# bmezaris/RetargetVid

Hardware: AMD Instinct MI355X
Metric: frames/sec end-to-end saliency+crop on 640x360 (higher is better)
Workload: dtype f32

## Files before the change

### retargetvid_amd/csrc/svc_net.hip

```cpp
#include <math.h>

#include <algorithm>

#include "svc_internal.h"
#include "svc_lanczos.h"
#include "svc_x3.h"

static inline int ceil_div(int a, int b) { return (a + b - 1) / b; }

__device__ __forceinline__ unsigned xcd_bx() {
    const unsigned b = blockIdx.x, n = gridDim.x;
    return (n & 7) ? b : (b & 7) * (n >> 3) + (b >> 3);
}

typedef float f32x2 __attribute__((ext_vector_type(2)));
__device__ __forceinline__ void fma4(float4 &a, const float4 x, const float4 w) {
    const f32x2 lo = __builtin_elementwise_fma((f32x2){x.x, x.y}, (f32x2){w.x, w.y}, (f32x2){a.x, a.y});
    const f32x2 hi = __builtin_elementwise_fma((f32x2){x.z, x.w}, (f32x2){w.z, w.w}, (f32x2){a.z, a.w});
    a = make_float4(lo.x, lo.y, hi.x, hi.y);
}


static thread_local char g_err[512] = "";
void svc_set_error(const char *fmt, ...) {
// ... 47 lines not shown
            const int ymin = vb[2 * y], cnt = vb[2 * y + 1];
            const int *k = vk + y * vks;
            const uint8_t *p = tile + (ymin - r_lo) * rowlen + i;
            int acc = 1 << (LZ_PREC - 1);
            for (int j = 0; j < cnt; ++j) acc += __mul24((int)p[j * rowlen], k[j]);
            dst[(size_t)(y - y0) * rowlen + i] = lc[min(max(acc >> LZ_PREC, 0), 255)];
        }
    }
}

#define STEM_TH 8
#define STEM_TW 16
#define STEM_PRS 100
__global__ __launch_bounds__(256) void k_stem_mfma(const float *__restrict__ X, const float *__restrict__ Wtr,
                                                   const float *__restrict__ bias, float *__restrict__ Y, int NH,
                                                   int NW, int OH, int OW, int tiles_x, int tiles_y) {
    constexpr int PR = 2 * STEM_TH + 1, PCW = 2 * STEM_TW + 1;
    __shared__ float Pin[PR * STEM_PRS];
    const int tid = threadIdx.x, lane = tid & 63, wave = tid >> 6, r = lane & 31, hh = lane >> 5;
    int bid = xcd_bx();
    const int tx = bid % tiles_x;
    bid /= tiles_x;
    const int ty = bid % tiles_y, f = bid / tiles_y;
    const int oy0 = ty * STEM_TH, ox0 = tx * STEM_TW, py0 = 2 * oy0 - 1, px0 = 2 * ox0 - 1;
    const float *xin = X + (size_t)f * NH * NW * 3;
    for (int idx = tid; idx < PR * PCW * 3; idx += 256) {
        const int pr = idx / (PCW * 3), rem = idx - pr * (PCW * 3), pc = rem / 3;
        const int y = py0 + pr, x = px0 + pc;
        float v = 0.f;
        if ((unsigned)y < (unsigned)NH && (unsigned)x < (unsigned)NW) v = xin[((long long)y * NW + px0) * 3 + rem];
        Pin[pr * STEM_PRS + rem] = v;
    }
    float4 wv[4];
#pragma unroll
    for (int q = 0; q < 4; ++q) wv[q] = *(const float4 *)(Wtr + r * 32 + 8 * q + 4 * hh);
    __syncthreads();
    const int p = 32 * wave + r, py = p / STEM_TW, px = p - py * STEM_TW;
    const float *src = Pin + (2 * py) * STEM_PRS + (2 * px) * 3;
    f32x16 acc;
#pragma unroll
    for (int i = 0; i < 16; ++i) acc[i] = 0.f;
#pragma unroll
    for (int q = 0; q < 4; ++q) {
        float t[4];
#pragma unroll
        for (int e = 0; e < 4; ++e) {
            const int k = 8 * q + 4 * hh + e;
            const int ky = (k * 57) >> 9;
            t[e] = k < 27 ? src[k + (STEM_PRS - 9) * ky] : 0.f;
        }
        acc = __builtin_amdgcn_mfma_f32_32x32x2f32(wv[q].x, t[0], acc, 0, 0, 0);
        acc = __builtin_amdgcn_mfma_f32_32x32x2f32(wv[q].y, t[1], acc, 0, 0, 0);
        acc = __builtin_amdgcn_mfma_f32_32x32x2f32(wv[q].z, t[2], acc, 0, 0, 0);
        acc = __builtin_amdgcn_mfma_f32_32x32x2f32(wv[q].w, t[3], acc, 0, 0, 0);
    }
    const int oy = oy0 + py, ox = ox0 + px;
    if (oy >= OH || ox >= OW) return;
    float *yp = Y + (((size_t)f * OH + oy) * OW + ox) * 32;
#pragma unroll
    for (int g = 0; g < 4; ++g) {
        const int c = 8 * g + 4 * hh;
        const float4 b = *(const float4 *)(bias + c);
        float4 v;
        v.x = fminf(fmaxf(acc[4 * g] + b.x, 0.f), 6.f);
        v.y = fminf(fmaxf(acc[4 * g + 1] + b.y, 0.f), 6.f);
        v.z = fminf(fmaxf(acc[4 * g + 2] + b.z, 0.f), 6.f);
        v.w = fminf(fmaxf(acc[4 * g + 3] + b.w, 0.f), 6.f);
        *(float4 *)(yp + c) = v;
    }
}

#define FR_TH 8
#define FR_TW 16
#define FR_HH (FR_TH + 2)
#define FR_HW (FR_TW + 2)
#define FR_NPX (FR_HH * FR_HW)
#define FR_PR (2 * FR_HH + 1)
#define FR_PC (2 * FR_HW + 1)
#define FR_PRS 112
#define FR_ES 36

#define FR_MAXT 32

struct FrontArgs {
    const uint8_t *frames;
    int h, w, NH, NW, OH, OW, tiles_x, tiles_y;
    const int *hb, *hk, *vb, *vk;
    int hks, vks;
    const float *lut;
    const float *Wstem, *bstem;
    const float *Wstem_l, *Wp_l;
    const float *Wd, *bd;
    const float *Wp, *bp;
    float *Y;
    float *in_dbg;
    int nr_cap, nc_cap;
    short row_lo[FR_MAXT], row_n[FR_MAXT], col_lo[FR_MAXT], col_n[FR_MAXT];
};

__host__ __device__ static inline int front_src_stride(int nc_cap) { return ((nc_cap * 3 + 6) >> 2) << 2; }
__host__ __device__ static inline int front_in_offset(int nr_cap, int nc_cap) {
    return (nr_cap * (front_src_stride(nc_cap) + FR_PRS) + 15) & ~15;
}
#define FR_IN_BYTES (FR_PR * FR_PRS * 4)
#define FR_SONLY_BYTES (FR_NPX * FR_ES * 4)
static inline int front_small_bytes(int nr_cap, int nc_cap) { return front_in_offset(nr_cap, nc_cap) + (FR_PR * 8 + 24 + 768) * 4; }
static inline int front_lds_bytes() { return FR_IN_BYTES + FR_SONLY_BYTES; }

__global__ __launch_bounds__(256) __attribute__((amdgpu_waves_per_eu(4, 8))) void k_front(const FrontArgs A) {
    extern __shared__ uint8_t sm_fr[];
    const int tid = threadIdx.x, lane = tid & 63, wave = tid >> 6, r = lane & 31, hh = lane >> 5;
    int bid = xcd_bx();
    const int tx = bid % A.tiles_x;
    bid /= A.tiles_x;
    const int ty = bid % A.tiles_y, f = bid / A.tiles_y;
    const int oy0 = ty * FR_TH, ox0 = tx * FR_TW, py0 = 2 * oy0 - 3, px0 = 2 * ox0 - 3;
    const int srs = front_src_stride(A.nc_cap);
    float *IN_s = (float *)sm_fr;
    float *S = (float *)(sm_fr + FR_IN_BYTES);
    uint8_t *src_s = (uint8_t *)S;
    uint8_t *tile_s = src_s + A.nr_cap * srs;
    int *vk_s = (int *)(src_s + front_in_offset(A.nr_cap, A.nc_cap));
    int *vb_s = vk_s + FR_PR * 8;
    float *lut_s = (float *)(vb_s + 24);
    float *D = S;
    const int c4 = tid & 7;
    const int ya = max(py0, 0), yb = min(py0 + FR_PR, A.NH), xa = max(px0, 0), xb = min(px0 + FR_PC, A.NW);
    const int r_lo = A.row_lo[ty], nr = A.row_n[ty], c_lo = A.col_lo[tx], nc3 = A.col_n[tx] * 3, ncol3 = (xb - xa) * 3;
    const uintptr_t g0 = (uintptr_t)A.frames + (((size_t)f * A.h + r_lo) * A.w + c_lo) * 3;
    const int rstep = A.w * 3, gm0 = (int)(g0 & 3), rs3 = rstep & 3;
    const int srow = tid >> 5, swi = tid & 31;
    uint32_t sv[4];
#pragma unroll
    for (int it = 0; it < 4; ++it) {
        const int row = srow + 8 * it;
        const uintptr_t ga = g0 + (size_t)row * rstep;
        const int nwords = ((int)(ga & 3) + nc3 + 3) >> 2;
        sv[it] = (row < nr && swi < nwords) ? *(const uint32_t *)((ga & ~(uintptr_t)3) + 4 * swi) : 0u;
    }
    const int ci = tid & 127, half = __builtin_amdgcn_readfirstlane(tid >> 7);
    const bool col_ok = ci < ncol3;
    const int xi = ci / 3, cc = ci - 3 * xi, x = min(xa + xi, A.NW - 1), pcol = (x - px0) * 3 + cc;
    const int xmin = A.hb[2 * x];
    int kh[8];
#pragma unroll
    for (int j = 0; j < 8; ++j) kh[j] = j < A.hks ? A.hk[x * A.hks + j] : 0;
    int vkv = 0, vbv = 0;
    if (tid < FR_PR * 8) {
        const int y = ya + (tid >> 3), j = tid & 7;
        if (y < yb && j < A.vks) vkv = A.vk[y * A.vks + j];
    } else if (tid < FR_PR * 8 + FR_PR) {
        const int y = ya + tid - FR_PR * 8;
        if (y < yb) vbv = A.vb[2 * y];
    }
    float lv[3];
#pragma unroll
    for (int i = 0; i < 3; ++i) lv[i] = A.lut[tid + 256 * i];
    for (int i = tid; i < FR_PR * FR_PRS / 4; i += 256) ((float4 *)IN_s)[i] = make_float4(0.f, 0.f, 0.f, 0.f);
#pragma unroll
    for (int it = 0; it < 4; ++it) {
        const int row = srow + 8 * it;
        if (row < nr && swi < (srs >> 2)) ((uint32_t *)src_s)[row * (srs >> 2) + swi] = sv[it];
    }
    if (tid < FR_PR * 8) vk_s[tid] = vkv;
    else if (tid < FR_PR * 8 + FR_PR) vb_s[tid - FR_PR * 8] = vbv;
#pragma unroll
    for (int i = 0; i < 3; ++i) lut_s[tid + 256 * i] = lv[i];
    __syncthreads();
    if (col_ok) {
        const uint8_t *p = src_s + (xmin - c_lo) * 3 + cc;
        for (int row = half; row < nr; row += 2) {
            const uint8_t *q = p + row * srs + ((gm0 + row * rs3) & 3);
            int acc = 1 << (LZ_PREC - 1);
#pragma unroll
            for (int j = 0; j < 8; ++j) acc += __mul24((int)q[3 * j], kh[j]);
            tile_s[row * FR_PRS + pcol] = (uint8_t)min(max(acc >> LZ_PREC, 0), 255);
        }
    }
    float4 wv[4];
#pragma unroll
    for (int q = 0; q < 4; ++q) wv[q] = *(const float4 *)(A.Wstem_l + (q * 64 + lane) * 4);
    __syncthreads();
    if (col_ok) {
        const float *lc = lut_s + cc * 256;
        const bool dbg_col = A.in_dbg && x >= 2 * ox0 && x < 2 * ox0 + 2 * FR_TW;
        for (int y = ya + half; y < yb; y += 2) {
            const int vrow = y - ya;
            const int4 k0 = *(const int4 *)(vk_s + vrow * 8), k1 = *(const int4 *)(vk_s + vrow * 8 + 4);
            const uint8_t *q = tile_s + (vb_s[vrow] - r_lo) * FR_PRS + pcol;
            int acc = 1 << (LZ_PREC - 1);
            acc += __mul24((int)q[0], k0.x) + __mul24((int)q[FR_PRS], k0.y) + __mul24((int)q[2 * FR_PRS], k0.z) + __mul24((int)q[3 * FR_PRS], k0.w);
            acc += __mul24((int)q[4 * FR_PRS], k1.x) + __mul24((int)q[5 * FR_PRS], k1.y) + __mul24((int)q[6 * FR_PRS], k1.z) + __mul24((int)q[7 * FR_PRS], k1.w);
            const float v = lc[min(max(acc >> LZ_PREC, 0), 255)];
            IN_s[(y - py0) * FR_PRS + pcol] = v;
            if (dbg_col && y >= 2 * oy0 && y < 2 * oy0 + 2 * FR_TH) A.in_dbg[(((size_t)f * A.NH + y) * A.NW + x) * 3 + cc] = v;
        }
    }
    __syncthreads();
    float4 wd[9];
#pragma unroll
    for (int t = 0; t < 9; ++t) wd[t] = *(const float4 *)(A.Wd + t * 32 + c4 * 4);
    for (int t = wave; t < (FR_NPX + 31) / 32; t += 4) {
        const int hp = t * 32 + r, hq = min(hp, FR_NPX - 1);
        const int hy = hq / FR_HW, hx = hq - hy * FR_HW;
        const float *src = IN_s + (2 * hy) * FR_PRS + (2 * hx) * 3;
        f32x16 acc;
#pragma unroll
        for (int i = 0; i < 16; ++i) acc[i] = 0.f;
#pragma unroll
        for (int q = 0; q < 4; ++q) {
            float tp[4];
#pragma unroll
            for (int e = 0; e < 4; ++e) {
                const int k = 8 * q + 4 * hh + e;
                const int ky = (k * 57) >> 9;
                tp[e] = k < 27 ? src[k + (FR_PRS - 9) * ky] : 0.f;
            }
            acc = __builtin_amdgcn_mfma_f32_32x32x2f32(wv[q].x, tp[0], acc, 0, 0, 0);
            acc = __builtin_amdgcn_mfma_f32_32x32x2f32(wv[q].y, tp[1], acc, 0, 0, 0);
            acc = __builtin_amdgcn_mfma_f32_32x32x2f32(wv[q].z, tp[2], acc, 0, 0, 0);
            acc = __builtin_amdgcn_mfma_f32_32x32x2f32(wv[q].w, tp[3], acc, 0, 0, 0);
        }
        if (hp < FR_NPX) {
            const bool in = (unsigned)(oy0 - 1 + hy) < (unsigned)A.OH && (unsigned)(ox0 - 1 + hx) < (unsigned)A.OW;
            float *sp = S + hp * FR_ES + 4 * hh;
#pragma unroll
            for (int g = 0; g < 4; ++g) {
                float4 v = make_float4(0.f, 0.f, 0.f, 0.f);
                if (in) {
                    const float4 b = *(const float4 *)(A.bstem + 8 * g + 4 * hh);
                    v.x = fminf(fmaxf(acc[4 * g] + b.x, 0.f), 6.f);
                    v.y = fminf(fmaxf(acc[4 * g + 1] + b.y, 0.f), 6.f);
                    v.z = fminf(fmaxf(acc[4 * g + 2] + b.z, 0.f), 6.f);
                    v.w = fminf(fmaxf(acc[4 * g + 3] + b.w, 0.f), 6.f);
                }
                *(float4 *)(sp + 8 * g) = v;
            }
        }
    }
    __syncthreads();
    float4 wq[4];
#pragma unroll
    for (int q = 0; q < 4; ++q) {
        wq[q] = *(const float4 *)(A.Wp_l + (q * 64 + lane) * 4);
        if (r >= 16) wq[q] = make_float4(0.f, 0.f, 0.f, 0.f);
    }
    {
        const float4 b = *(const float4 *)(A.bd + c4 * 4);
        const int oy = tid >> 5, ox = ((tid >> 3) & 3) * 4;
        float4 a4[4];
#pragma unroll
        for (int i = 0; i < 4; ++i) a4[i] = make_float4(0.f, 0.f, 0.f, 0.f);
#pragma unroll
        for (int ky = 0; ky < 3; ++ky) {
            const float *sp = S + ((oy + ky) * FR_HW + ox) * FR_ES + c4 * 4;
            float4 xv[6];
#pragma unroll
            for (int j = 0; j < 6; ++j) xv[j] = *(const float4 *)(sp + j * FR_ES);
#pragma unroll
            for (int kx = 0; kx < 3; ++kx) {
                const float4 w = wd[ky * 3 + kx];
#pragma unroll
                for (int i = 0; i < 4; ++i) fma4(a4[i], xv[i + kx], w);
            }
        }
        __syncthreads();
#pragma unroll
        for (int i = 0; i < 4; ++i) {
            float4 o;
            o.x = fminf(fmaxf(a4[i].x + b.x, 0.f), 6.f);
            o.y = fminf(fmaxf(a4[i].y + b.y, 0.f), 6.f);
            o.z = fminf(fmaxf(a4[i].z + b.z, 0.f), 6.f);
            o.w = fminf(fmaxf(a4[i].w + b.w, 0.f), 6.f);
            *(float4 *)(D + (oy * FR_TW + ox + i) * FR_ES + c4 * 4) = o;
        }
    }
    __syncthreads();
    {
        f32x16 a0, a1;
#pragma unroll
        for (int i = 0; i < 16; ++i) { a0[i] = 0.f; a1[i] = 0.f; }
        const int px = 32 * wave + r;
        const float *dp = D + px * FR_ES + 4 * hh;
#pragma unroll
        for (int q = 0; q < 4; ++q) {
            const float4 a = *(const float4 *)(dp + 8 * q);
            if (q < 2) {
                a0 = __builtin_amdgcn_mfma_f32_32x32x2f32(wq[q].x, a.x, a0, 0, 0, 0);
                a0 = __builtin_amdgcn_mfma_f32_32x32x2f32(wq[q].y, a.y, a0, 0, 0, 0);
                a0 = __builtin_amdgcn_mfma_f32_32x32x2f32(wq[q].z, a.z, a0, 0, 0, 0);
                a0 = __builtin_amdgcn_mfma_f32_32x32x2f32(wq[q].w, a.w, a0, 0, 0, 0);
            } else {
                a1 = __builtin_amdgcn_mfma_f32_32x32x2f32(wq[q].x, a.x, a1, 0, 0, 0);
                a1 = __builtin_amdgcn_mfma_f32_32x32x2f32(wq[q].y, a.y, a1, 0, 0, 0);
                a1 = __builtin_amdgcn_mfma_f32_32x32x2f32(wq[q].z, a.z, a1, 0, 0, 0);
                a1 = __builtin_amdgcn_mfma_f32_32x32x2f32(wq[q].w, a.w, a1, 0, 0, 0);
            }
        }
        const int oy = oy0 + (px >> 4), ox = ox0 + (px & 15);
        if (oy < A.OH && ox < A.OW) {
            float *yp = A.Y + (((size_t)f * A.OH + oy) * A.OW + ox) * 16;
#pragma unroll
            for (int g = 0; g < 2; ++g) {
                const int col = 8 * g + 4 * hh;
// ... 579 lines not shown
    __shared__ unsigned rmax[BP_ROWS];
    const int tid = threadIdx.x;
    const int y0 = blockIdx.x * BP_ROWS, y1 = min(h, y0 + BP_ROWS);
    if (tid < BP_ROWS) rmax[tid] = 0u;
    __syncthreads();
    for (int c0 = 0; c0 < w; c0 += 256 * BP_COLS) {
        unsigned cmax[BP_COLS];
#pragma unroll
        for (int j = 0; j < BP_COLS; ++j) cmax[j] = 0u;
        for (int y = y0; y < y1; ++y) {
            unsigned r = 0u;
#pragma unroll
            for (int j = 0; j < BP_COLS; ++j) {
                const int c = c0 + j * 256 + tid;
                if (c < w) {
                    const unsigned v = load(y, c);
                    cmax[j] = max(cmax[j], v);
                    r = max(r, v);
                }
            }
            r = max(r, (unsigned)__shfl_xor((int)r, 32)); r = max(r, (unsigned)__shfl_xor((int)r, 16));
            r = max(r, (unsigned)__shfl_xor((int)r, 8)); r = max(r, (unsigned)__shfl_xor((int)r, 4));
            r = max(r, (unsigned)__shfl_xor((int)r, 2)); r = max(r, (unsigned)__shfl_xor((int)r, 1));
            if ((tid & 63) == 0 && r) atomicMax(&rmax[y - y0], r);
        }
#pragma unroll
        for (int j = 0; j < BP_COLS; ++j) {
            const int c = c0 + j * 256 + tid;
            if (c < w && cmax[j]) atomicMax(prof + h + c, cmax[j]);
        }
    }
    __syncthreads();
    if (tid < y1 - y0 && rmax[tid]) atomicMax(prof + y0 + tid, rmax[tid]);
}

__global__ __launch_bounds__(256) void k_border_profile(const uint8_t *__restrict__ maps, int h, int w, unsigned *__restrict__ profile) {
    const size_t f = blockIdx.y;
    const uint8_t *m = maps + f * (size_t)h * w;
    border_band([&](int y, int c) { return (unsigned)m[(size_t)y * w + c]; }, h, w, profile + f * (size_t)(h + w));
}

__global__ __launch_bounds__(256) void k_quantise_profile(const float *__restrict__ pre, const unsigned *__restrict__ fmax,
                                                          uint8_t *__restrict__ out, int h, int w, int thr,
                                                          unsigned long long *__restrict__ census, unsigned *__restrict__ rows,
                                                          unsigned *__restrict__ profile) {
    const uint32_t f = blockIdx.y;
    const size_t base = (size_t)f * h * w;
    const float m = dec_f32(fmax[f]);
    border_band([&](int y, int c) {
        const size_t gid = base + (size_t)y * w + c;
        const float e = expf(pre[gid] - m);
        const uint8_t v = (uint8_t)(e * 255.0f);
        out[gid] = (int)v < thr ? (uint8_t)0 : v;
        if (census && thr > 0) {
            const int d = (int)v - (thr - 1);
            if (d >= 0 && d <= 2) {
                atomicAdd((unsigned *)(census + 4) + f * 4 + d, 1u);
                if (rows) atomicAdd(rows + f * 4 + d, 1u);
            }
        }
        return (unsigned)v;
    }, h, w, profile + (size_t)f * (h + w));
}

enum Buf { B_IN, B_P0, B_P1, B_E0, B_E1, B_F4X, B_F2X, B_CAT1, B_PCD, B_PC, B_CAT2, B_U2E, B_U2, B_CAT3, B_P3E, B_DEC,
           B_LOGIT, B_PRE, B_T1, B_T2, B_COUNT };

static const struct { int div, ch; } BUF_SHAPE[B_COUNT] = {
    {1, 3}, {2, 32}, {2, 32}, {0, 0}, {0, 0}, {8, 64}, {16, 160},
    {32, 1296}, {32, 1296}, {32, 256},
    {16, 384}, {16, 768}, {16, 128},
    {8, 192}, {8, 384}, {8, 64},
    {0, 0}, {0, 0}, {32, 768}, {16, 384}};
static size_t buf_floats(int NH, int NW, int b) { return (size_t)(NH / BUF_SHAPE[b].div) * (NW / BUF_SHAPE[b].div) * BUF_SHAPE[b].ch; }

#define LZ_ROWS 8
#define SD_ROWS 7

struct NetPlan {
    int h = 0, w = 0, NH = 0, NW = 0, nb = 0;
    size_t off[B_COUNT + 1];
    DevBuf ws, fmax, lut, gauss;
    DevBuf hb, hk, vb, vk;
    int hks = 0, vks = 0, lz_tile_cap = 0;
    int fr_nr = 0, fr_nc = 0;
    bool fr_ok = false;
    short fr_row_lo[32], fr_row_n[32], fr_col_lo[32], fr_col_n[32];
    int sd_tile_cap = 0;
    int last_n = 0;
    bool last_front = false;
    int gauss_filled = 0;
    float *buf(int b) const { return (float *)ws.p + off[b] * (size_t)nb; }
    size_t per_frame(int b) const { return off[b + 1] - off[b]; }
};

static void optimal_out_size(int h, int w, int &NH, int &NW) {
    double ar = (double)h / w, best = -1.0;
    int b1 = 8, b2 = 13;
    for (int n1 = 7; n1 < 14; ++n1)
        for (int n2 = 7; n2 < 14; ++n2)
            if (n1 * n2 >= 100 && n1 * n2 <= 120) {
                double t = (double)n1 / n2;
                double ratio = std::min(ar, t) / std::max(ar, t);
                if (ratio > best) { best = ratio; b1 = n1; b2 = n2; }
            }
    NH = b1 * 32;
    NW = b2 * 32;
}

static void linspace01(int steps, std::vector<float> &v) {
    v.resize(steps);
    if (steps == 1) { v[0] = 0.f; return; }
    float step = 1.0f / (float)(steps - 1);
    int half = steps / 2;
    for (int i = 0; i < steps; ++i) v[i] = (i < half) ? (0.f + step * i) : (1.f - step * (steps - 1 - i));
}

static int build_plan(SvcHandle *h, int height, int width, int nb) {
    NetPlan *p = h->plan;
    if (!p) p = h->plan = new NetPlan();
    if (p->h == height && p->w == width && p->nb >= nb) return SVC_OK;
    p->gauss_filled = 0;
    int NH, NW;
    optimal_out_size(height, width, NH, NW);
    const bool same_size = (p->h == height && p->w == width);
    p->h = height; p->w = width; p->NH = NH; p->NW = NW; p->nb = nb;
    const size_t H1 = NH / 2, W1 = NW / 2, H2 = NH / 4, W2 = NW / 4, H3 = NH / 8, W3 = NW / 8, H4 = NH / 16,
                 W4 = NW / 16, H5 = NH / 32, W5 = NW / 32;
    size_t sz[B_COUNT];
    for (int b = 0; b < B_COUNT; ++b) sz[b] = BUF_SHAPE[b].div ? buf_floats(NH, NW, b) : 0;
    sz[B_E0] = std::max(std::max(H1 * W1 * 96, H2 * W2 * 144), std::max(H3 * W3 * 192, std::max(H4 * W4 * 576, H5 * W5 * 960)));
    sz[B_E1] = std::max(std::max(H1 * W1 * 32, H2 * W2 * 144), std::max(H3 * W3 * 192, std::max(H4 * W4 * 576, H5 * W5 * 960)));
    sz[B_LOGIT] = (H3 * W3 + 3) / 4 * 4;
    sz[B_PRE] = ((size_t)height * width + 3) / 4 * 4;
    p->off[0] = 0;
    for (int b = 0; b < B_COUNT; ++b) p->off[b + 1] = p->off[b] + (sz[b] + 3) / 4 * 4;
    int rc = p->ws.ensure(p->off[B_COUNT] * (size_t)nb * sizeof(float));
    if (rc) return rc;
    rc = p->fmax.ensure((size_t)nb * sizeof(unsigned));
    if (rc) return rc;
    if (same_size) return SVC_OK;
    std::vector<int> hb, hk, vb, vk;
    lanczos_tab(width, NW, hb, hk, p->hks);
    lanczos_tab(height, NH, vb, vk, p->vks);
    int cap = 0;
    for (int y0 = 0; y0 < NH; y0 += LZ_ROWS) {
        int y1 = std::min(NH, y0 + LZ_ROWS);
        cap = std::max(cap, vb[2 * (y1 - 1)] + vb[2 * (y1 - 1) + 1] - vb[2 * y0]);
    }
    p->lz_tile_cap = cap;
    p->fr_nr = p->fr_nc = 0;
    const int fty = ceil_div(NH / 2, FR_TH), ftx = ceil_div(NW / 2, FR_TW);
    p->fr_ok = p->hks <= 8 && p->vks <= 8 && fty <= FR_MAXT && ftx <= FR_MAXT;
    for (int t = 0; t < FR_MAXT; ++t) p->fr_row_lo[t] = p->fr_row_n[t] = p->fr_col_lo[t] = p->fr_col_n[t] = 0;
    for (int t = 0; t < fty && p->fr_ok; ++t) {
        const int ya = std::max(2 * t * FR_TH - 3, 0), yb = std::min(2 * t * FR_TH - 3 + FR_PR, NH);
        p->fr_row_lo[t] = (short)vb[2 * ya];
        p->fr_row_n[t] = (short)(vb[2 * (yb - 1)] + vb[2 * (yb - 1) + 1] - vb[2 * ya]);
        p->fr_nr = std::max(p->fr_nr, (int)p->fr_row_n[t]);
    }
    for (int t = 0; t < ftx && p->fr_ok; ++t) {
        const int xa = std::max(2 * t * FR_TW - 3, 0), xb = std::min(2 * t * FR_TW - 3 + FR_PC, NW);
        p->fr_col_lo[t] = (short)hb[2 * xa];
        p->fr_col_n[t] = (short)(hb[2 * (xb - 1)] + hb[2 * (xb - 1) + 1] - hb[2 * xa]);
        p->fr_nc = std::max(p->fr_nc, (int)p->fr_col_n[t]);
    }
    p->fr_ok = p->fr_ok && p->fr_nr <= 32 && front_src_stride(p->fr_nc) <= 128 &&
               front_small_bytes(p->fr_nr, p->fr_nc) <= FR_SONLY_BYTES;
    if ((rc = p->hb.ensure(hb.size() * 4)) || (rc = p->hk.ensure(hk.size() * 4)) || (rc = p->vb.ensure(vb.size() * 4)) ||
        (rc = p->vk.ensure(vk.size() * 4)))
        return rc;
    SVC_HIP(hipMemcpy(p->hb.p, hb.data(), hb.size() * 4, hipMemcpyHostToDevice));
    SVC_HIP(hipMemcpy(p->hk.p, hk.data(), hk.size() * 4, hipMemcpyHostToDevice));
    SVC_HIP(hipMemcpy(p->vb.p, vb.data(), vb.size() * 4, hipMemcpyHostToDevice));
    SVC_HIP(hipMemcpy(p->vk.p, vk.data(), vk.size() * 4, hipMemcpyHostToDevice));
    std::vector<float> lut(3 * 256);
    const float mean[3] = {0.485f, 0.456f, 0.406f}, sd[3] = {0.229f, 0.224f, 0.225f};
    for (int c = 0; c < 3; ++c)
        for (int v = 0; v < 256; ++v) {
            volatile float t = (float)v / 255.0f;
            volatile float d = t - mean[c];
            lut[c * 256 + v] = d / sd[c];
        }
    if ((rc = p->lut.ensure(lut.size() * 4))) return rc;
    SVC_HIP(hipMemcpy(p->lut.p, lut.data(), lut.size() * 4, hipMemcpyHostToDevice));
    std::vector<float> ys, xs, g(H5 * W5 * 16);
    linspace01((int)H5, ys);
    linspace01((int)W5, xs);
    for (int i = 0; i < 16; ++i) {
        const float *gp = h->gauss_params.data() + i * 4;
        float sy = expf(gp[1]), sx = expf(gp[3]);
        for (size_t y = 0; y < H5; ++y)
            for (size_t x = 0; x < W5; ++x) {
                float dy = (ys[y] - gp[0]) / sy, dx = (xs[x] - gp[2]) / sx;
                float m = 1.0f;
                m *= expf(-(dy * dy) / 2.0f);
                m *= expf(-(dx * dx) / 2.0f);
                g[(y * W5 + x) * 16 + i] = m * 6.0f;
            }
    }
    if ((rc = p->gauss.ensure(g.size() * 4))) return rc;
    SVC_HIP(hipMemcpy(p->gauss.p, g.data(), g.size() * 4, hipMemcpyHostToDevice));
    float scy = (float)NH / (float)height;
    cap = 0;
    for (int oy0 = 0; oy0 < height; oy0 += SD_ROWS) {
        int oy1 = std::min(height, oy0 + SD_ROWS);
        int ylo = (int)std::max(scy * (oy0 + 0.5f) - 0.5f, 0.f);
        int yhi = std::min((int)std::max(scy * ((oy1 - 1) + 0.5f) - 0.5f, 0.f) + 1, NH - 1);
        cap = std::max(cap, yhi - ylo + 1);
    }
    p->sd_tile_cap = cap;
    return SVC_OK;
}

int svc_net_release(SvcHandle *h) {
    if (h->plan) {
        NetPlan *p = h->plan;
        p->ws.release(); p->fmax.release(); p->lut.release(); p->gauss.release();
        p->hb.release(); p->hk.release(); p->vb.release(); p->vk.release();
        delete p;
        h->plan = nullptr;
    }
    for (auto &kv : h->cvtabs) kv.second.release();
    h->cvtabs.clear();
    for (auto &kv : h->lztabs) { kv.second.bounds.release(); kv.second.coeff.release(); }
    h->lztabs.clear();
    return SVC_OK;
}

#define RC(x) do { int rc_ = (x); if (rc_) return rc_; } while (0)

static inline unsigned blocks256(size_t total) { return (unsigned)((total + 255) / 256); }

static int raise_lds_limit(SvcHandle *h, const void *kfn, int bytes) {
    if (h->lds_attr_done.insert(kfn).second) SVC_HIP(hipFuncSetAttribute(kfn, hipFuncAttributeMaxDynamicSharedMemorySize, bytes));
    return SVC_OK;
}

__global__ void k_lane_weights(const float *__restrict__ Wt, int ldw, int nsteps, int tiles, int nrows, float4 *__restrict__ out) {
    const size_t i = (size_t)blockIdx.x * 256 + threadIdx.x;
    if (i >= (size_t)nsteps * tiles * 64) return;
    const int lane = (int)(i & 63), tile = (int)((i >> 6) % tiles), st = (int)((i >> 6) / tiles);
    out[i] = *(const float4 *)(Wt + (size_t)min(tile * 32 + (lane & 31), nrows - 1) * ldw + 8 * st + 4 * (lane >> 5));
}

enum WForm { X3_ROWS = 0, X3_LANES = 1, F32_LANES = 2, W_MATRIX = 3 };
__global__ void k_x3_weights(const float *__restrict__ Wt, int ldw, int K, int Q, int tiles, int nrows, int order, uint4 *__restrict__ out) {
    const size_t i = (size_t)blockIdx.x * 256 + threadIdx.x;
    if (i >= (size_t)tiles * 32 * Q * 2) return;
    int n, q, hh;
    if (order == X3_ROWS) { hh = (int)(i & 1); q = (int)((i >> 1) % Q); n = (int)((i >> 1) / Q); }
    else { const int lane = (int)(i & 63); hh = lane >> 5; const size_t t = i >> 6; n = (int)(t % tiles) * 32 + (lane & 31); q = (int)(t / tiles); }
    const float *w = Wt + (size_t)min(n, nrows - 1) * ldw;
    float v[8];
#pragma unroll
    for (int j = 0; j < 8; ++j) {
        const int k = 16 * q + 8 * (j >> 2) + 4 * hh + (j & 3);
        v[j] = k < K ? w[k] : 0.f;
    }
    const X3 s = x3_split<true>(make_float4(v[0], v[1], v[2], v[3]), make_float4(v[4], v[5], v[6], v[7]));
    X3Q H, Mi, L;
    H.v = s.h; Mi.v = s.m; L.v = s.l;
    out[i * 3] = H.q; out[i * 3 + 1] = Mi.q; out[i * 3 + 2] = L.q;
}

static int weight_copy(SvcHandle *h, hipStream_t s, WForm form, const float *Wt, int ldw, int K, int Npad, const void **out) {
    *out = Wt;
    if (form == W_MATRIX) return SVC_OK;
    const auto key = std::make_tuple((const void *)Wt, ldw, K, Npad, (int)form);
    auto it = h->w_copies.find(key);
    if (it == h->w_copies.end()) {
        DevBuf b;
        const int tiles = (Npad + 31) >> 5, nsteps = K >> 3, Q = (K + 15) >> 4;
        const size_t cells = form == F32_LANES ? (size_t)nsteps * tiles * 64 : (size_t)tiles * 32 * Q * 2;
        RC(b.ensure(cells * (form == F32_LANES ? sizeof(float4) : 3 * sizeof(uint4))));
        if (form == F32_LANES) k_lane_weights<<<blocks256(cells), 256, 0, s>>>(Wt, ldw, nsteps, tiles, Npad, (float4 *)b.p);
        else k_x3_weights<<<blocks256(cells), 256, 0, s>>>(Wt, ldw, K, Q, tiles, Npad, form, (uint4 *)b.p);
        SVC_CHECK_LAUNCH();
        SVC_HIP(hipStreamSynchronize(s));
        it = h->w_copies.emplace(key, b).first;
    }
    *out = it->second.p;
    return SVC_OK;
}

static WForm lane_form(const SvcHandle *h, int K) {
    return h->mx && (K & 15) == 0 ? X3_LANES : h->sk_lane && (K & 7) == 0 ? F32_LANES : W_MATRIX;
}

#define PWR_NT 2
#define PW_SK_MAX_WG 2048

using PwrFn = decltype(&k_pwr<8, false>);
template <int KS, bool UPS>
static PwrFn pwr_kfn(bool mx) { return mx ? k_pwr<KS, UPS, true> : k_pwr<KS, UPS>; }

static int launch_pw_ex(SvcHandle *h, hipStream_t s, const float *X, int ldx, const float *Wt, int ldw, int K,
                        const float *bias, int relu6v, int N, const float *R, int ldr, float *Y, int ldy, int M, int n,
                        const UpsAdd *ups) {
    ProfScope ps(h, SVC_K_PW, s);
    const int Npad = (N + 31) / 32 * 32, tiles = Npad / 32;
    UpsAdd ua = ups ? *ups : UpsAdd{nullptr, 0, 0, 0, make_fdiv(1), make_fdiv(1)};
// ... 807 lines not shown
        return;
    }
#pragma unroll
    for (int j = 0; j < 2; ++j) {
        const int tile = t0 + 4 * j;
        if (tile >= ptiles) continue;
        const int pm = tile % MP, nt = tile / MP;
        const int px = pm * 32 + r;
        const int oy = oy0 + px / TOW, ox = ox0 + px % TOW;
        if (oy >= OH || ox >= OW) continue;
        const size_t pix = ((size_t)f * OH + oy) * OW + ox;
#pragma unroll
        for (int g = 0; g < 4; ++g) {
            const int col = nt * 32 + 8 * g + 4 * hh;
            if (col >= Cout) continue;
            const float4 bv = *(const float4 *)(bp + col);
            float4 v = make_float4(acc[j][4 * g] + bv.x, acc[j][4 * g + 1] + bv.y, acc[j][4 * g + 2] + bv.z, acc[j][4 * g + 3] + bv.w);
            if (R) {
                const float4 rv = *(const float4 *)(R + pix * Cout + col);
                v.x += rv.x; v.y += rv.y; v.z += rv.z; v.w += rv.w;
            }
            *(float4 *)(Y + pix * ldy + col) = v;
        }
    }
}

template <int S, int TOH, int TOW, bool EXP, int CI, int CE, int CO, bool MX>
static int launch_irb_as(SvcHandle *h, hipStream_t s, const float *X, int n, int H, int W, const InvRes &B, const float *R, float *Y) {
    const int Cin = B.inp, Ce = B.dw.cout, Cout = B.oup, CoutP = (Cout + 31) / 32 * 32, OH = H / S, OW = W / S;
    const void *We = EXP ? B.expand.w.dev : nullptr, *Wp = B.project.w.dev;
    if (MX) {
        RC(weight_copy(h, s, X3_ROWS, B.expand.w.dev, Cin, Cin, (Ce + 31) / 32 * 32, &We));
        if (Cout == 64) RC(weight_copy(h, s, X3_ROWS, B.project.w.dev, Ce, Ce, CoutP, &Wp));
    }
    const int tx = ceil_div(OW, TOW), ty = ceil_div(OH, TOH);
    const size_t lds = IrbGeom<S, TOH, TOW>::lds_floats(Cin, CoutP, EXP, Ce, IRB_XREG && EXP && CI > 0 && CI <= 32 && (CI % 8) == 0, MX) * 4;
    const auto kfn = k_irb<S, TOH, TOW, EXP, CI, CE, CO, MX>;
    RC(raise_lds_limit(h, (const void *)kfn, 120 * 1024));
    kfn<<<dim3((unsigned)(n * tx * ty)), 256, lds, s>>>(X, H, W, Cin, (const float *)We, EXP ? B.expand.b.dev : nullptr, Ce, B.dw.w.dev, B.dw.b.dev,
                                                        (const float *)Wp, B.project.b.dev, Cout, CoutP, R, Y, Cout, OH, OW, tx, ty);
    SVC_CHECK_LAUNCH();
    return SVC_OK;
}
using IrbFn = decltype(&launch_irb_as<1, 8, 8, false, 32, 32, 16, false>);
template <int S, int TOH, int TOW, int CI, int CE, int CO>
static IrbFn irb_on_pipe(bool mx) { return mx ? launch_irb_as<S, TOH, TOW, true, CI, CE, CO, true> : launch_irb_as<S, TOH, TOW, true, CI, CE, CO, false>; }

static int launch_irb(SvcHandle *h, hipStream_t s, const float *X, int n, int H, int W, const InvRes &B, int stride, const float *R, float *Y) {
    ProfScope ps(h, SVC_K_PW, s);
    const int Cin = B.inp, Ce = B.dw.cout, Cout = B.oup;
    const bool mx = h->mx != 0;
    IrbFn fn = nullptr;
    if (!B.has_expand) {
        if (Cin == 32 && Ce == 32 && Cout == 16) fn = launch_irb_as<1, 8, 8, false, 32, 32, 16, false>;
        else {
            svc_set_error("no k_irb instance for a %d -> %d -> %d block without expansion", Cin, Ce, Cout);
            return SVC_E_INVALID;
        }
    } else if (stride == 2 && Cin == 16 && Ce == 96 && Cout == 24) fn = irb_on_pipe<2, 4, 8, 16, 96, 24>(mx);
    else if (stride == 2 && Cin == 24 && Ce == 144 && Cout == 32) fn = launch_irb_as<2, 4, 8, true, 24, 144, 32, false>;
    else if (stride == 1 && Cin == 24 && Ce == 144 && Cout == 24) fn = irb_on_pipe<1, 8, 8, 24, 144, 24>(mx);
    else if (stride == 1 && Cin == 32 && Ce == 192 && Cout == 32) fn = irb_on_pipe<1, 8, 8, 32, 192, 32>(mx);
    else if (stride == 1 && Cin == 32 && Ce == 192 && Cout == 64) fn = irb_on_pipe<1, 8, 8, 32, 192, 64>(mx);
    else {
        svc_set_error("no k_irb instance for a stride-%d %d -> %d -> %d block", stride, Cin, Ce, Cout);
        return SVC_E_INVALID;
    }
    return fn(h, s, X, n, H, W, B, R, Y);
}


static int net_front(SvcHandle *h, hipStream_t s, const uint8_t *frames, int n, float *stem_out, float *y) {
    NetPlan *p = h->plan;
    const NetGraph &g = h->net;
    const InvRes &B = g.block[0];
    const int NH = p->NH, NW = p->NW, H = NH / 2, W = NW / 2;
    float *IN = p->buf(B_IN);
    p->last_front = h->front && p->fr_ok;
    if (p->last_front) {
        ProfScope ps(h, SVC_K_STEM, s);
        FrontArgs A;
        A.frames = frames; A.h = p->h; A.w = p->w; A.NH = NH; A.NW = NW; A.OH = H; A.OW = W;
        A.tiles_x = ceil_div(W, FR_TW); A.tiles_y = ceil_div(H, FR_TH);
        A.hb = (const int *)p->hb.p; A.hk = (const int *)p->hk.p; A.vb = (const int *)p->vb.p; A.vk = (const int *)p->vk.p;
        A.hks = p->hks; A.vks = p->vks; A.lut = (const float *)p->lut.p;
        A.Wstem = (const float *)h->stem_wt.p; A.bstem = g.stem.b.dev;
        const void *wl;
        RC(weight_copy(h, s, F32_LANES, (const float *)h->stem_wt.p, 32, 32, 32, &wl));
        A.Wstem_l = (const float *)wl;
        RC(weight_copy(h, s, F32_LANES, B.project.w.dev, 32, 32, 16, &wl));
        A.Wp_l = (const float *)wl;
        A.Wd = B.dw.w.dev; A.bd = B.dw.b.dev; A.Wp = B.project.w.dev; A.bp = B.project.b.dev;
        A.Y = y; A.in_dbg = h->keep_input ? IN : nullptr;
        A.nr_cap = p->fr_nr; A.nc_cap = p->fr_nc;
        for (int i = 0; i < FR_MAXT; ++i) {
            A.row_lo[i] = p->fr_row_lo[i]; A.row_n[i] = p->fr_row_n[i];
            A.col_lo[i] = p->fr_col_lo[i]; A.col_n[i] = p->fr_col_n[i];
        }
        k_front<<<dim3((unsigned)(n * A.tiles_x * A.tiles_y)), 256, front_lds_bytes(), s>>>(A);
        SVC_CHECK_LAUNCH();
        return SVC_OK;
    }
    {
        ProfScope ps(h, SVC_K_LANCZOS, s);
        dim3 grid(ceil_div(NH, LZ_ROWS), n);
        size_t lds = ((size_t)p->lz_tile_cap * p->w * 3 + 15) / 16 * 16 + ((size_t)p->lz_tile_cap * NW * 3 + 15) / 16 * 16 +
                     (size_t)NW * p->hks * 4 + 768 * 4;
        k_lanczos_norm<<<grid, 256, lds, s>>>(frames, IN, p->h, p->w, NH, NW, (const int *)p->hb.p, (const int *)p->hk.p,
                                             p->hks, (const int *)p->vb.p, (const int *)p->vk.p, p->vks,
                                             (const float *)p->lut.p, LZ_ROWS, p->lz_tile_cap);
        SVC_CHECK_LAUNCH();
    }
    {
        ProfScope ps(h, SVC_K_STEM, s);
        const int tx = ceil_div(W, STEM_TW), ty = ceil_div(H, STEM_TH);
        k_stem_mfma<<<dim3((unsigned)(n * tx * ty)), 256, 0, s>>>(IN, (const float *)h->stem_wt.p, g.stem.b.dev, stem_out, NH, NW,
                                                                 H, W, tx, ty);
        SVC_CHECK_LAUNCH();
    }
    return launch_irb(h, s, stem_out, n, H, W, B, 1, nullptr, y);
}

static int dw_project(SvcHandle *h, hipStream_t s, const float *X, const InvRes &B, const float *R, int ldr, float *dw_out, float *Y,
                      int n, int H, int W) {
    if (H * W >= dwpw_min_px(h)) return launch_dwpw(h, s, X, B.dw, B.project, R, ldr, Y, B.oup, n, H, W);
    RC(launch_dw(h, s, X, B.dw, dw_out, n, H, W));
    return launch_pw(h, s, dw_out, B.dw.cout, B.project, R, ldr, Y, B.oup, n * H * W, n);
}

static int backbone_block(SvcHandle *h, hipStream_t s, int idx, const float *x, float *out, int n, int &H, int &W) {
    NetPlan *p = h->plan;
    const InvRes &B = h->net.block[idx - 1];
    const float *res = (B.stride == 1 && B.inp == B.oup) ? x : nullptr;
    const bool tap = (idx == 7 || idx == 14);
    const int dws = (B.stride == 2 && !tap) ? 2 : 1;
    int OH = H / dws, OW = W / dws;
    float *y = tap ? p->buf(idx == 7 ? B_F4X : B_F2X) : out;
    if (idx <= 7) RC(launch_irb(h, s, x, n, H, W, B, dws, res, y));
    else {
        const float *dwin = x;
        if (B.has_expand) {
            dwin = p->buf(B_E0);
            RC(launch_pw(h, s, x, B.inp, B.expand, nullptr, 0, p->buf(B_E0), B.dw.cin, n * H * W, n));
        }
        RC(dw_project(h, s, dwin, B, res, B.oup, p->buf(B_E1), y, n, H, W));
    }
    if (tap) {
        ProfScope ps(h, SVC_K_RESAMPLE, s);
        k_subsample<<<blocks256((size_t)n * (OH / 2) * (OW / 2) * (B.oup / 4)), 256, 0, s>>>(y, out, n, OH, OW, B.oup);
        SVC_CHECK_LAUNCH();
        OH /= 2; OW /= 2;
    }
    H = OH; W = OW;
    return SVC_OK;
}

static int head_f18(SvcHandle *h, hipStream_t s, const float *x, int n, int H5, int W5) {
    return launch_pw(h, s, x, 320, h->net.f18, nullptr, 0, h->plan->buf(B_CAT1), 1296, n * H5 * W5, n);
}

static int head_skip_2x(SvcHandle *h, hipStream_t s, int n, int H5, int W5) {
    NetPlan *p = h->plan;
    return launch_pwpw(h, s, p->buf(B_F2X), 160, h->net.skip2x_expand, h->net.skip2x_reduce, p->buf(B_CAT2) + 256, 384, n * 4 * H5 * W5);
}

static int head_skip_4x(SvcHandle *h, hipStream_t s, int n, int H5, int W5) {
    NetPlan *p = h->plan;
    return launch_pwpw(h, s, p->buf(B_F4X), 64, h->net.skip4x_expand, h->net.skip4x_reduce, p->buf(B_CAT3) + 128, 192, n * 16 * H5 * W5);
// ... 516 lines not shown
```

Baseline: 25630.

## Precompute packed per-tile Lanczos tables and use sliding-window vertical resample in front kernel

Moves the per-column horizontal resampling metadata (source offset, column, channel, x) and its 7 taps into a host-built packed table indexed by tile, and the vertical taps plus base row into 8-int records read through the constant address space with scalar mad24. The vertical pass now splits the rows into contiguous halves per thread group and keeps a sliding window of 7 source bytes, advancing it by at most one row, which removes LDS staging of vk/vb and the repeated index math. Kernel taps are cut from 8 to 7, the last stem MFMA is skipped, and the fast path now requires at most 7 taps and unit-step vertical bases, so other configurations fall back to the slower path.

```diff
diff --git a/retargetvid_amd/csrc/svc_net.hip b/retargetvid_amd/csrc/svc_net.hip
--- a/retargetvid_amd/csrc/svc_net.hip
+++ b/retargetvid_amd/csrc/svc_net.hip
@@ -153,11 +153,20 @@
 
 #define FR_MAXT 32
 
+typedef int i32x8 __attribute__((ext_vector_type(8)));
+typedef __attribute__((address_space(4))) const i32x8 FrVRec;
+
+__device__ static inline int mad24_s(int byte, int coef, int acc) {
+    int r;
+    asm("v_mad_i32_i24 %0, %1, %2, %3" : "=v"(r) : "v"(byte), "s"(coef), "v"(acc));
+    return r;
+}
+
 struct FrontArgs {
     const uint8_t *frames;
     int h, w, NH, NW, OH, OW, tiles_x, tiles_y;
-    const int *hb, *hk, *vb, *vk;
-    int hks, vks;
+    const int4 *ht;
+    const int *vt;
     const float *lut;
     const float *Wstem, *bstem;
     const float *Wstem_l, *Wp_l;
@@ -175,7 +184,7 @@
 }
 #define FR_IN_BYTES (FR_PR * FR_PRS * 4)
 #define FR_SONLY_BYTES (FR_NPX * FR_ES * 4)
-static inline int front_small_bytes(int nr_cap, int nc_cap) { return front_in_offset(nr_cap, nc_cap) + (FR_PR * 8 + 24 + 768) * 4; }
+static inline int front_small_bytes(int nr_cap, int nc_cap) { return front_in_offset(nr_cap, nc_cap) + 768 * 4; }
 static inline int front_lds_bytes() { return FR_IN_BYTES + FR_SONLY_BYTES; }
 
 __global__ __launch_bounds__(256) __attribute__((amdgpu_waves_per_eu(4, 8))) void k_front(const FrontArgs A) {
@@ -185,19 +194,17 @@
     const int tx = bid % A.tiles_x;
     bid /= A.tiles_x;
     const int ty = bid % A.tiles_y, f = bid / A.tiles_y;
-    const int oy0 = ty * FR_TH, ox0 = tx * FR_TW, py0 = 2 * oy0 - 3, px0 = 2 * ox0 - 3;
+    const int oy0 = ty * FR_TH, ox0 = tx * FR_TW, py0 = 2 * oy0 - 3;
     const int srs = front_src_stride(A.nc_cap);
     float *IN_s = (float *)sm_fr;
     float *S = (float *)(sm_fr + FR_IN_BYTES);
     uint8_t *src_s = (uint8_t *)S;
     uint8_t *tile_s = src_s + A.nr_cap * srs;
-    int *vk_s = (int *)(src_s + front_in_offset(A.nr_cap, A.nc_cap));
-    int *vb_s = vk_s + FR_PR * 8;
-    float *lut_s = (float *)(vb_s + 24);
+    float *lut_s = (float *)(src_s + front_in_offset(A.nr_cap, A.nc_cap));
     float *D = S;
     const int c4 = tid & 7;
-    const int ya = max(py0, 0), yb = min(py0 + FR_PR, A.NH), xa = max(px0, 0), xb = min(px0 + FR_PC, A.NW);
-    const int r_lo = A.row_lo[ty], nr = A.row_n[ty], c_lo = A.col_lo[tx], nc3 = A.col_n[tx] * 3, ncol3 = (xb - xa) * 3;
+    const int ya = max(py0, 0), yb = min(py0 + FR_PR, A.NH);
+    const int r_lo = A.row_lo[ty], nr = A.row_n[ty], c_lo = A.col_lo[tx], nc3 = A.col_n[tx] * 3;
     const uintptr_t g0 = (uintptr_t)A.frames + (((size_t)f * A.h + r_lo) * A.w + c_lo) * 3;
     const int rstep = A.w * 3, gm0 = (int)(g0 & 3), rs3 = rstep & 3;
     const int srow = tid >> 5, swi = tid & 31;
@@ -210,20 +217,10 @@
         sv[it] = (row < nr && swi < nwords) ? *(const uint32_t *)((ga & ~(uintptr_t)3) + 4 * swi) : 0u;
     }
     const int ci = tid & 127, half = __builtin_amdgcn_readfirstlane(tid >> 7);
-    const bool col_ok = ci < ncol3;
-    const int xi = ci / 3, cc = ci - 3 * xi, x = min(xa + xi, A.NW - 1), pcol = (x - px0) * 3 + cc;
-    const int xmin = A.hb[2 * x];
-    int kh[8];
-#pragma unroll
-    for (int j = 0; j < 8; ++j) kh[j] = j < A.hks ? A.hk[x * A.hks + j] : 0;
-    int vkv = 0, vbv = 0;
-    if (tid < FR_PR * 8) {
-        const int y = ya + (tid >> 3), j = tid & 7;
-        if (y < yb && j < A.vks) vkv = A.vk[y * A.vks + j];
-    } else if (tid < FR_PR * 8 + FR_PR) {
-        const int y = ya + tid - FR_PR * 8;
-        if (y < yb) vbv = A.vb[2 * y];
-    }
+    const int4 h0 = A.ht[(tx * 2) * 128 + ci], h1 = A.ht[(tx * 2 + 1) * 128 + ci];
+    const bool col_ok = h0.x < 0;
+    const int poff = h0.x & 255, pcol = (h0.x >> 8) & 127, cc = (h0.x >> 15) & 3, x = (h0.x >> 17) & 1023;
+    const int kh[7] = {h0.y, h0.z, h0.w, h1.x, h1.y, h1.z, h1.w};
     float lv[3];
 #pragma unroll
     for (int i = 0; i < 3; ++i) lv[i] = A.lut[tid + 256 * i];
@@ -233,18 +230,16 @@
         const int row = srow + 8 * it;
         if (row < nr && swi < (srs >> 2)) ((uint32_t *)src_s)[row * (srs >> 2) + swi] = sv[it];
     }
-    if (tid < FR_PR * 8) vk_s[tid] = vkv;
-    else if (tid < FR_PR * 8 + FR_PR) vb_s[tid - FR_PR * 8] = vbv;
 #pragma unroll
     for (int i = 0; i < 3; ++i) lut_s[tid + 256 * i] = lv[i];
     __syncthreads();
     if (col_ok) {
-        const uint8_t *p = src_s + (xmin - c_lo) * 3 + cc;
+        const uint8_t *p = src_s + poff;
         for (int row = half; row < nr; row += 2) {
             const uint8_t *q = p + row * srs + ((gm0 + row * rs3) & 3);
             int acc = 1 << (LZ_PREC - 1);
 #pragma unroll
-            for (int j = 0; j < 8; ++j) acc += __mul24((int)q[3 * j], kh[j]);
+            for (int j = 0; j < 7; ++j) acc += __mul24((int)q[3 * j], kh[j]);
             tile_s[row * FR_PRS + pcol] = (uint8_t)min(max(acc >> LZ_PREC, 0), 255);
         }
     }
@@ -255,16 +250,39 @@
     if (col_ok) {
         const float *lc = lut_s + cc * 256;
         const bool dbg_col = A.in_dbg && x >= 2 * ox0 && x < 2 * ox0 + 2 * FR_TW;
-        for (int y = ya + half; y < yb; y += 2) {
-            const int vrow = y - ya;
-            const int4 k0 = *(const int4 *)(vk_s + vrow * 8), k1 = *(const int4 *)(vk_s + vrow * 8 + 4);
-            const uint8_t *q = tile_s + (vb_s[vrow] - r_lo) * FR_PRS + pcol;
-            int acc = 1 << (LZ_PREC - 1);
-            acc += __mul24((int)q[0], k0.x) + __mul24((int)q[FR_PRS], k0.y) + __mul24((int)q[2 * FR_PRS], k0.z) + __mul24((int)q[3 * FR_PRS], k0.w);
-            acc += __mul24((int)q[4 * FR_PRS], k1.x) + __mul24((int)q[5 * FR_PRS], k1.y) + __mul24((int)q[6 * FR_PRS], k1.z) + __mul24((int)q[7 * FR_PRS], k1.w);
-            const float v = lc[min(max(acc >> LZ_PREC, 0), 255)];
-            IN_s[(y - py0) * FR_PRS + pcol] = v;
+        const int ymid = ya + ((yb - ya + 1) >> 1), y0 = half ? ymid : ya, y1 = half ? yb : ymid;
+        const FrVRec *vt = (const FrVRec *)A.vt;
+        const uint8_t *col = tile_s + pcol;
+        float *dst = IN_s + pcol - py0 * FR_PRS;
+        auto emit = [&](int y, float v) {
+            dst[y * FR_PRS] = v;
             if (dbg_col && y >= 2 * oy0 && y < 2 * oy0 + 2 * FR_TH) A.in_dbg[(((size_t)f * A.NH + y) * A.NW + x) * 3 + cc] = v;
+        };
+        if (y0 < y1) {
+            i32x8 rc = vt[y0];
+            int s = rc[7] - r_lo, wd7[7];
+#pragma unroll
+            for (int j = 0; j < 7; ++j) wd7[j] = col[(s + j) * FR_PRS];
+            auto sum_and_advance = [&](int ynext) {
+                const i32x8 nx = vt[min(ynext, A.NH - 1)];
+                const int nb = col[(s + 7) * FR_PRS];
+                int acc = 1 << (LZ_PREC - 1);
+#pragma unroll
+                for (int j = 0; j < 7; ++j) acc = mad24_s(wd7[j], rc[j], acc);
+                const bool adv = nx[7] - r_lo != s;
+#pragma unroll
+                for (int j = 0; j < 6; ++j) wd7[j] = adv ? wd7[j + 1] : wd7[j];
+                wd7[6] = adv ? nb : wd7[6];
+                s += adv;
+                rc = nx;
+                return min(max(acc >> LZ_PREC, 0), 255);
+            };
+            int idx = sum_and_advance(y0 + 1);
+            for (int y = y0; y < y1; ++y) {
+                const float v = lc[idx];
+                idx = sum_and_advance(y + 2);
+                emit(y, v);
+            }
         }
     }
     __syncthreads();
@@ -290,7 +308,7 @@
             acc = __builtin_amdgcn_mfma_f32_32x32x2f32(wv[q].x, tp[0], acc, 0, 0, 0);
             acc = __builtin_amdgcn_mfma_f32_32x32x2f32(wv[q].y, tp[1], acc, 0, 0, 0);
             acc = __builtin_amdgcn_mfma_f32_32x32x2f32(wv[q].z, tp[2], acc, 0, 0, 0);
-            acc = __builtin_amdgcn_mfma_f32_32x32x2f32(wv[q].w, tp[3], acc, 0, 0, 0);
+            if (q < 3) acc = __builtin_amdgcn_mfma_f32_32x32x2f32(wv[q].w, tp[3], acc, 0, 0, 0);
         }
         if (hp < FR_NPX) {
             const bool in = (unsigned)(oy0 - 1 + hy) < (unsigned)A.OH && (unsigned)(ox0 - 1 + hx) < (unsigned)A.OW;
@@ -1036,6 +1054,8 @@
     size_t off[B_COUNT + 1];
     DevBuf ws, fmax, lut, gauss;
     DevBuf hb, hk, vb, vk;
+    DevBuf fr_vt;
+    DevBuf fr_ht;
     int hks = 0, vks = 0, lz_tile_cap = 0;
     int fr_nr = 0, fr_nc = 0;
     bool fr_ok = false;
@@ -1105,7 +1125,8 @@
     p->lz_tile_cap = cap;
     p->fr_nr = p->fr_nc = 0;
     const int fty = ceil_div(NH / 2, FR_TH), ftx = ceil_div(NW / 2, FR_TW);
-    p->fr_ok = p->hks <= 8 && p->vks <= 8 && fty <= FR_MAXT && ftx <= FR_MAXT;
+    p->fr_ok = p->hks <= 7 && p->vks <= 7 && fty <= FR_MAXT && ftx <= FR_MAXT;
+    for (int y = 1; y < NH && p->fr_ok; ++y) p->fr_ok = vb[2 * y] - vb[2 * (y - 1)] <= 1;
     for (int t = 0; t < FR_MAXT; ++t) p->fr_row_lo[t] = p->fr_row_n[t] = p->fr_col_lo[t] = p->fr_col_n[t] = 0;
     for (int t = 0; t < fty && p->fr_ok; ++t) {
         const int ya = std::max(2 * t * FR_TH - 3, 0), yb = std::min(2 * t * FR_TH - 3 + FR_PR, NH);
@@ -1128,6 +1149,28 @@
     SVC_HIP(hipMemcpy(p->hk.p, hk.data(), hk.size() * 4, hipMemcpyHostToDevice));
     SVC_HIP(hipMemcpy(p->vb.p, vb.data(), vb.size() * 4, hipMemcpyHostToDevice));
     SVC_HIP(hipMemcpy(p->vk.p, vk.data(), vk.size() * 4, hipMemcpyHostToDevice));
+    if (p->fr_ok) {
+        std::vector<int> vt((size_t)NH * 8, 0);
+        for (int y = 0; y < NH; ++y) {
+            for (int j = 0; j < p->vks; ++j) vt[y * 8 + j] = vk[(size_t)y * p->vks + j];
+            vt[y * 8 + 7] = vb[2 * y];
+        }
+        if ((rc = p->fr_vt.ensure(vt.size() * 4))) return rc;
+        SVC_HIP(hipMemcpy(p->fr_vt.p, vt.data(), vt.size() * 4, hipMemcpyHostToDevice));
+        std::vector<int> ht((size_t)ftx * 2 * 128 * 4, 0);
+        for (int t = 0; t < ftx; ++t) {
+            const int px0 = 2 * t * FR_TW - 3, xa = std::max(px0, 0), xb = std::min(px0 + FR_PC, NW);
+            for (int ci = 0; ci < (xb - xa) * 3; ++ci) {
+                const int x = xa + ci / 3, cc = ci % 3;
+                const int poff = (hb[2 * x] - p->fr_col_lo[t]) * 3 + cc, pcol = (x - px0) * 3 + cc;
+                int *r0 = &ht[((size_t)(t * 2) * 128 + ci) * 4], *r1 = r0 + 128 * 4;
+                r0[0] = (int)(0x80000000u | (unsigned)poff | (unsigned)pcol << 8 | (unsigned)cc << 15 | (unsigned)x << 17);
+                for (int j = 0; j < p->hks; ++j) (j < 3 ? r0[1 + j] : r1[j - 3]) = hk[(size_t)x * p->hks + j];
+            }
+        }
+        if ((rc = p->fr_ht.ensure(ht.size() * 4))) return rc;
+        SVC_HIP(hipMemcpy(p->fr_ht.p, ht.data(), ht.size() * 4, hipMemcpyHostToDevice));
+    }
     std::vector<float> lut(3 * 256);
     const float mean[3] = {0.485f, 0.456f, 0.406f}, sd[3] = {0.229f, 0.224f, 0.225f};
     for (int c = 0; c < 3; ++c)
@@ -1171,7 +1214,7 @@
     if (h->plan) {
         NetPlan *p = h->plan;
         p->ws.release(); p->fmax.release(); p->lut.release(); p->gauss.release();
-        p->hb.release(); p->hk.release(); p->vb.release(); p->vk.release();
+        p->hb.release(); p->hk.release(); p->vb.release(); p->vk.release(); p->fr_vt.release(); p->fr_ht.release();
         delete p;
         h->plan = nullptr;
     }
@@ -2145,8 +2188,8 @@
         FrontArgs A;
         A.frames = frames; A.h = p->h; A.w = p->w; A.NH = NH; A.NW = NW; A.OH = H; A.OW = W;
         A.tiles_x = ceil_div(W, FR_TW); A.tiles_y = ceil_div(H, FR_TH);
-        A.hb = (const int *)p->hb.p; A.hk = (const int *)p->hk.p; A.vb = (const int *)p->vb.p; A.vk = (const int *)p->vk.p;
-        A.hks = p->hks; A.vks = p->vks; A.lut = (const float *)p->lut.p;
+        A.ht = (const int4 *)p->fr_ht.p; A.vt = (const int *)p->fr_vt.p;
+        A.lut = (const float *)p->lut.p;
         A.Wstem = (const float *)h->stem_wt.p; A.bstem = g.stem.b.dev;
         const void *wl;
         RC(weight_copy(h, s, F32_LANES, (const float *)h->stem_wt.p, 32, 32, 32, &wl));
```

After: 26050, median of 6. 1.6% higher.
